# gaoxiang12/ORB-YGZ-SLAM

Hardware: AMD Instinct MI355X
Metric: frames/s ORB extract+match, 752x480 8-lvl 1000-feat; 1->8 GPU scaling (higher is better)
Workload: dtype u8

## Files before the change

### include/ygzf.h

```cpp
#ifndef YGZF_H
#define YGZF_H
#include <stddef.h>
#include <stdint.h>

#ifdef __cplusplus
extern "C" {
#endif

typedef enum ygzf_status {
    YGZF_OK = 0,
    YGZF_ERR_INVALID = -1,
    YGZF_ERR_NO_DEVICE = -2,
    YGZF_ERR_HIP = -3,
    YGZF_ERR_UNSUPPORTED = -4,
    YGZF_ERR_STATE = -5
} ygzf_status;

typedef struct ygzf_ctx ygzf_ctx;

typedef struct ygzf_extractor_cfg {
    int nfeatures;
    float scale_factor;
    int nlevels;
    int ini_th_fast;
    int min_th_fast;
    int cv_mode;
} ygzf_extractor_cfg;

typedef enum ygzf_cv_mode { YGZF_CV_LEGACY_SSE2 = 0, YGZF_CV_LEGACY_INT = 1, YGZF_CV_4 = 2 } ygzf_cv_mode;

typedef struct ygzf_kp {
    float x, y, size, angle, response;
    int32_t octave, class_id;
} ygzf_kp;

int ygzf_create(int device, const ygzf_extractor_cfg *cfg, int max_width, int max_height, int max_batch, ygzf_ctx **out);
void ygzf_destroy(ygzf_ctx *ctx);
const char *ygzf_last_error(const ygzf_ctx *ctx);

int ygzf_scale_tables_host(const ygzf_extractor_cfg *cfg, float *scale, float *inv_scale, float *sigma2, float *inv_sigma2, int *nfeat);
int ygzf_pyramid_plan_host(const ygzf_extractor_cfg *cfg, int w, int h, int *n_strips, int *lds_bytes, int *level_wh, unsigned short *rows, int rows_cap);
int ygzf_pyramid_plan_base_host(const ygzf_extractor_cfg *cfg, int w, int h);
int ygzf_octree_sort_plan_host(const ygzf_extractor_cfg *cfg, int w, int h, int *groups, int groups_cap);

int ygzf_extract_resident(ygzf_ctx *ctx, ygzf_kp *kps, uint8_t *desc, int cap, int *n_out);

int ygzf_device_mem_info(ygzf_ctx *ctx, size_t *free_bytes, size_t *total_bytes);

enum ygzf_fast_plan { YGZF_FAST_PLAN_AUTO = 0, YGZF_FAST_PLAN_ONE_PASS = 1, YGZF_FAST_PLAN_INI_FIRST = 2 };
int ygzf_set_fast_plan(ygzf_ctx *ctx, int plan);
int ygzf_get_fast_plan(const ygzf_ctx *ctx, int *plan);
enum ygzf_fast_kernel { YGZF_FAST_KERNEL_AUTO = 0, YGZF_FAST_KERNEL_REGISTER_STAGING = 1, YGZF_FAST_KERNEL_CELL_TABLE = 2 };
int ygzf_set_fast_kernel(ygzf_ctx *ctx, int kernel);
int ygzf_get_fast_stats(const ygzf_ctx *ctx, float *corner_quads_per_pass, float *passes_per_cell);
int ygzf_phase_clocks(ygzf_ctx *ctx, int kernel, unsigned long long *out16, int reset);
int ygzf_set_extract_ahead(ygzf_ctx *ctx, int on);
int ygzf_set_carry_previous(ygzf_ctx *ctx, int on);

int ygzf_get_levels(const ygzf_ctx *ctx);
int ygzf_get_scale_tables(const ygzf_ctx *ctx, float *scale, float *inv_scale, float *sigma2, float *inv_sigma2);
int ygzf_get_features_per_level(const ygzf_ctx *ctx, int *nfeat);
int ygzf_level_size(const ygzf_ctx *ctx, int w, int h, int level, int *lw, int *lh);
int ygzf_host_row_pitch(int w);
int ygzf_max_keypoints(const ygzf_ctx *ctx, int w, int h);

int ygzf_compute_pyramid(ygzf_ctx *ctx, const uint8_t *img, int w, int h, int stride, uint8_t *const *levels_out);

int ygzf_extract(ygzf_ctx *ctx, const uint8_t *img, int w, int h, int stride, ygzf_kp *kps, uint8_t *desc, int cap, int *n_out);

int ygzf_extract_batch_device(ygzf_ctx *ctx, const uint8_t *d_imgs, int n_frames, int w, int h, int row_pitch, size_t frame_stride);
int ygzf_extract_batch_host(ygzf_ctx *ctx, const uint8_t *imgs, int n_frames, int w, int h, int row_pitch, size_t frame_stride);
int ygzf_extract_batch_host_frames(ygzf_ctx *ctx, const uint8_t *const *frames, int n_frames, int w, int h, int row_pitch);
int ygzf_batch_counts(ygzf_ctx *ctx, int *n_kp );
int ygzf_batch_fetch(ygzf_ctx *ctx, int frame, ygzf_kp *kps, uint8_t *desc, int cap, int *n_out);
int ygzf_batch_fetch_all(ygzf_ctx *ctx, ygzf_kp *kps, uint8_t *desc, int *n_kp, int stride);
int ygzf_batch_fetch_packed(ygzf_ctx *ctx, void *host, size_t host_bytes, size_t *off_kps, size_t *off_desc, int *row_entries, size_t *bytes_out);
// ... 187 lines not shown
```

### orb_ygz_slam_amd/capi.py

```python
import ctypes as C
import os

import numpy as np

from . import build as _build

KP_DTYPE = np.dtype([("x", "<f4"), ("y", "<f4"), ("size", "<f4"), ("angle", "<f4"), ("response", "<f4"),
                     ("octave", "<i4"), ("class_id", "<i4")])
assert KP_DTYPE.itemsize == 28


class YgzfError(RuntimeError):
    pass


class ExtractorCfg(C.Structure):
    _fields_ = [("nfeatures", C.c_int), ("scale_factor", C.c_float), ("nlevels", C.c_int), ("ini_th_fast", C.c_int),
                ("min_th_fast", C.c_int), ("cv_mode", C.c_int)]


CV_LEGACY_SSE2, CV_LEGACY_INT, CV_4 = 0, 1, 2


class Camera(C.Structure):
# ... 193 lines not shown
def host_row_pitch(w):
    return load_library().ygzf_host_row_pitch(int(w))


def pyramid_plan_host(nfeatures, scale_factor, nlevels, w, h):
    L = load_library()
    cfg = ExtractorCfg(nfeatures, scale_factor, nlevels, 20, 7, 0)
    n, lds = C.c_int(0), C.c_int(0)
    wh = np.zeros(2 * nlevels, np.int32)
    rows = np.zeros(64 * nlevels * 4, np.uint16)
    rc = L.ygzf_pyramid_plan_host(C.byref(cfg), w, h, C.byref(n), C.byref(lds), _p(wh), _p(rows), rows.size)
    if rc != 0:
        raise YgzfError("ygzf_pyramid_plan_host failed (%d)" % rc)
    L.ygzf_pyramid_plan_base_host.argtypes = [C.c_void_p, C.c_int, C.c_int]
    base = L.ygzf_pyramid_plan_base_host(C.byref(cfg), w, h)
    if base < 0:
        raise YgzfError("ygzf_pyramid_plan_base_host failed (%d)" % base)
    return {"strips": n.value, "base": base, "lds_bytes": lds.value, "levels": [(int(wh[2 * l]), int(wh[2 * l + 1])) for l in range(nlevels)],
            "rows": rows[:n.value * nlevels * 4].astype(np.int64).reshape(n.value, nlevels, 4)}


def octree_sort_plan_host(nfeatures, scale_factor, nlevels, w, h):
    L = load_library()
    L.ygzf_octree_sort_plan_host.argtypes = [C.POINTER(ExtractorCfg), C.c_int, C.c_int, C.c_void_p, C.c_int]
    cfg = ExtractorCfg(nfeatures, scale_factor, nlevels, 20, 7, 0)
    out = np.zeros(6 * 16, np.int32)
    n = L.ygzf_octree_sort_plan_host(C.byref(cfg), w, h, _p(out), out.size)
    if n < 0:
        raise YgzfError("ygzf_octree_sort_plan_host failed (%d)" % n)
    keys = ("l0", "n", "block", "cap", "lds_cand", "lds_bytes")
    return [dict(zip(keys, (int(v) for v in out[6 * i:6 * i + 6]))) for i in range(n)]


class Extractor:

    def __init__(self, nfeatures=1000, scale_factor=1.2, nlevels=8, ini_th=20, min_th=7, max_width=752, max_height=480,
                 max_batch=1, device=0, cv_mode=CV_LEGACY_SSE2):
        self.L = load_library()
        self.nlevels = nlevels
        self.cfg = ExtractorCfg(nfeatures, scale_factor, nlevels, ini_th, min_th, cv_mode)
        self._wh = (max_width, max_height, 0)
        self.max_width, self.max_height = max_width, max_height
        self._inflight = []
        self.h = C.c_void_p()
        rc = self.L.ygzf_create(device, C.byref(self.cfg), max_width, max_height, max_batch, C.byref(self.h))
        if rc != 0:
            self.h = C.c_void_p()
            raise YgzfError("ygzf_create failed (%d): %s" % (rc, self.L.ygzf_last_error(None).decode()))

    def close(self):
        if getattr(self, "h", None) and self.h.value:
            self.L.ygzf_destroy(self.h)
            self.h = C.c_void_p()

    def __del__(self):
        try:
            self.close()
        except Exception:
            pass

    def _ck(self, rc):
        if rc < 0:
            raise YgzfError("libygzf error %d: %s" % (rc, self.L.ygzf_last_error(self.h).decode()))
        return rc

    def tables(self):
# ... 796 lines not shown
```

### orb_ygz_slam_amd/csrc/kernels.h

```cpp
#ifndef YGZF_KERNELS_H
#define YGZF_KERNELS_H
#include "ygzf_internal.h"

namespace ygzf {

hipError_t upload_constants(const int *umax16);

struct PyrTabs {
    const int *xofs;
    const short *xalpha;
    const int *yofs;
    const short *ybeta;
    const PyrColRec *cols;
    const PyrRowRec *rows;
    const PyrTileRec *tiles;
};
void launch_pyr_resize(hipStream_t st, const FrameSet &fs, const LevelGeom *dGeom, const LevelGeom &g, int level, int nFrames, const PyrTabs &T);
constexpr int kPyrFolds = 4;
__host__ __device__ constexpr int pyr_fold_chunks(int foldLog2) { return foldLog2 == 0 ? 21 : foldLog2 == 1 ? 11 : foldLog2 == 2 ? 6 : 3; }
__host__ __device__ constexpr int pyr_fold_pitch(int foldLog2) { return 16 * pyr_fold_chunks(foldLog2); }
__host__ __device__ constexpr int pyr_fold_rows(int foldLog2) { return foldLog2 == 0 ? 44 : foldLog2 == 1 ? 84 : foldLog2 == 2 ? 166 : 330; }
constexpr int kPyrTileRows = 32;
void launch_repitch_rows(hipStream_t st, const uint8_t *src, size_t srcPitch, uint8_t *dst, size_t dstPitch, int w, size_t rows);
constexpr int kHostFrameListMax = 128;
// ... 98 lines not shown
    const float *mpProjX, *mpProjY, *mpProjXR, *mpViewCos, *mpAngle;
    const int *mpLevel;
    float nnratio;
    int maxDist;
    float fx, fy, cx, cy, mb, mbf, minX, minY, maxX, maxY, gridInvW, gridInvH;
    float scaleFactors[kMaxLevels];
    float th;
    int bMono, checkLevel, checkOri;
    uint8_t *owner;
    int *match;
    int *nmatches;
    int *match12;
    int capCur, capLast, descInLds, qpInLds;
    int spill;
    int specDeep;
    void *spillScratch;
    long long spillStride;
    void *qpScratch;
    long long *dbg;
    int handoverFence;
    int fixedLanes;
    int unitWorld;
    int serialOrder;
    int split;
    int *splitCnt;
    unsigned char *splitX;
    unsigned *matchStat;
};
constexpr int kMatchStatFallbacks = 0, kMatchStatRoundCap = 1, kMatchStatExtRoom = 2, kMatchStatExtended = 3, kMatchStatRescans = 4, kMatchStatWords = 5;
constexpr int kMatchCauseRounds = 1, kMatchCauseExtRoom = 2;
constexpr int kSpillSpec = 1, kSpillMisc = 2;
constexpr int kMatchSplitRec = 56;
size_t match_lds_bytes(int capCur, int capLast, bool descInLds, int spill, size_t *spillBytes, bool specDeep);
hipError_t match_prepare(size_t ldsBytes);
void launch_backproject_unit(hipStream_t st, const ygzf_kp *keys, const int *cnt, long long kpStride, int maxKp, int nFrames, float fx,
                             float fy, float cx, float cy, float *world);
void launch_match_last(hipStream_t st, const MatchArgs &A, int nPairs, size_t ldsBytes);


void launch_bow(hipStream_t st, int nNodes, const int *kfOff, const int *kfIdx, const int *fOff, const int *fIdx, const uint8_t *kfValid,
                const ygzf_kp *kfKeys, const uint8_t *kfDesc, int nF, const ygzf_kp *fKeys, const uint8_t *fDesc, float nnratio, int checkOri, int *match,
                unsigned char *binOf, int *hist, int *nmatches);

struct TriArgs {
    int nEntries, nNodes, n1;
    const int *off1, *idx1, *off2, *idx2;
    const ygzf_kp *keys1, *keys2;
    const uint8_t *desc1, *desc2, *hasMp1, *hasMp2;
    const float *uR1, *uR2;
    const float *sf2, *sigma2;
    float F[9];
    float ex, ey;
    int onlyStereo, checkOri;
    int *match12;
    unsigned char *binOf;
    int *hist, *nmatches;
};
void launch_triangulation(hipStream_t st, const TriArgs &A);

struct FrustumArgs {
    int n;
    const uint8_t *candidate;
    const float *world, *normal, *maxDistInv, *minDistInv, *mfMaxDistance;
    float Rcw[9], tcw[3], Ow[3];
    float fx, fy, cx, cy, mbf, minX, minY, maxX, maxY;
    float viewingCosLimit;
// ... 167 lines not shown
```

### orb_ygz_slam_amd/csrc/match_kernels.hip

```cpp
#include "kernels.h"
#include "wave_ops.h"

namespace ygzf {

constexpr int GRID_COLS = 64, GRID_ROWS = 48, GRID_CELLS = GRID_COLS * GRID_ROWS;
constexpr int TH_HIGH = 100;
constexpr int HISTO_LENGTH = 30;

__device__ __forceinline__ int m_lane() { return threadIdx.x & 63; }

__device__ __forceinline__ int m_wave_incl_scan(int v) { return wave_incl_scan(v); }

__global__ void k_backproject_unit(const ygzf_kp *__restrict__ keys, const int *__restrict__ cnt, long long kpStride, float fx,
                                   float fy, float cx, float cy, float *__restrict__ world) {
    const int f = blockIdx.y;
    const int i = blockIdx.x * blockDim.x + threadIdx.x;
    if (i >= cnt[f]) return;
    const ygzf_kp k = keys[(long long) f * kpStride + i];
    float *w = world + ((long long) f * kpStride + i) * 3;
    w[0] = (k.x - cx) / fx;
    w[1] = (k.y - cy) / fy;
    w[2] = 1.f;
}

struct QueryParam {
    float u, v, radius, ur, angle;
    unsigned char minCx, maxCx, minCy, maxCy;
    signed char minLevel, maxLevel;
    unsigned char valid, hasObs;
    unsigned pad;
};

constexpr int kMatchBlock = 1024;
constexpr unsigned kNoKey = (256u << 16);
constexpr int kExtSlots = 64;

typedef unsigned v4u_t __attribute__((ext_vector_type(4)));
typedef __attribute__((address_space(3))) const v4u_t lds_uint4_t;
__device__ __forceinline__ void lds_desc(const unsigned long long *base, int i2, unsigned long long &d0, unsigned long long &d1, unsigned long long &d2,
                                         unsigned long long &d3) {
    lds_uint4_t *p = (lds_uint4_t *) (base + 4 * (size_t) i2);
    const v4u_t a = p[0], b = p[1];
    d0 = ((unsigned long long) a.y << 32) | a.x; d1 = ((unsigned long long) a.w << 32) | a.z;
    d2 = ((unsigned long long) b.y << 32) | b.x; d3 = ((unsigned long long) b.w << 32) | b.z;
}

struct MatchLds {
    int *cellStart, *cellFill, *list, *events;
    QueryParam *qp;
    unsigned long long *desc;
    float *cx, *cy, *cang;
    uint4 *specKey;
    ushort4 *specI2;
    uint4 *specKeyB;
    ushort4 *specI2B;
    float *qang;
    unsigned char *qobs;
    unsigned char *owner, *octave;
    int *match;
    int *claim;
    unsigned char *extOf;
    unsigned *extKey;
    unsigned short *extI2;
    int *extWork;
};

__device__ __forceinline__ unsigned wave_min_dpp(unsigned v) {
    unsigned t;
    t = (unsigned) __builtin_amdgcn_update_dpp((int) v, (int) v, 0xb1, 0xf, 0xf, false); v = t < v ? t : v;
    t = (unsigned) __builtin_amdgcn_update_dpp((int) v, (int) v, 0x4e, 0xf, 0xf, false); v = t < v ? t : v;
    t = (unsigned) __builtin_amdgcn_update_dpp((int) v, (int) v, 0x124, 0xf, 0xf, false); v = t < v ? t : v;
    t = (unsigned) __builtin_amdgcn_update_dpp((int) v, (int) v, 0x128, 0xf, 0xf, false); v = t < v ? t : v;
    const unsigned a = (unsigned) __builtin_amdgcn_readlane((int) v, 0), b = (unsigned) __builtin_amdgcn_readlane((int) v, 16);
    const unsigned c = (unsigned) __builtin_amdgcn_readlane((int) v, 32), d = (unsigned) __builtin_amdgcn_readlane((int) v, 48);
    const unsigned ab = a < b ? a : b, cd = c < d ? c : d;
    return ab < cd ? ab : cd;
}

#if (defined(__gfx950__) || defined(__gfx942__)) && !defined(YGZF_FORCE_HANDOVER_FENCE)
constexpr bool kHandoverScopedAccess = true;
#else
// ... 162 lines not shown
    for (int st = 4; st >= 1; st >>= 1)
#pragma unroll
        for (int e = 0; e < 8; e++)
            if ((e & st) == 0 && K[e + st] < K[e]) {
                const unsigned tk = K[e], tj = J[e];
                K[e] = K[e + st]; J[e] = J[e + st];
                K[e + st] = tk; J[e + st] = tj;
            }
}

template <int kXor>
__device__ __forceinline__ void spec_merge8_xor(unsigned (&K)[8], unsigned (&J)[8], int lane) {
    const int addr = (lane ^ kXor) << 2;
    unsigned pk[8], pj[8];
#pragma unroll
    for (int e = 0; e < 8; e++) {
        pk[e] = (unsigned) __builtin_amdgcn_ds_bpermute(addr, (int) K[7 - e]);
        pj[e] = (unsigned) __builtin_amdgcn_ds_bpermute(addr, (int) J[7 - e]);
    }
#pragma unroll
    for (int e = 0; e < 8; e++)
        if (pk[e] < K[e]) { K[e] = pk[e]; J[e] = pj[e]; }
#pragma unroll
    for (int st = 4; st >= 1; st >>= 1)
#pragma unroll
        for (int e = 0; e < 8; e++)
            if ((e & st) == 0 && K[e + st] < K[e]) {
                const unsigned tk = K[e], tj = J[e];
                K[e] = K[e + st]; J[e] = J[e + st];
                K[e + st] = tk; J[e + st] = tj;
            }
}

__global__ __launch_bounds__(kMatchBlock) void k_match_last(MatchArgs A) {
    extern __shared__ __attribute__((aligned(16))) unsigned char dyn[];
    __shared__ int s_tmp[20];
    __shared__ int s_hist[HISTO_LENGTH];
    const int tid = threadIdx.x, lane = m_lane(), wave = tid >> 6;
    const int S = A.split > 1 ? A.split : 1;
    const int pair = S > 1 ? (int) blockIdx.x / S : (int) blockIdx.x, part = (int) blockIdx.x - pair * S;
    const int nt = A.curCnt[(long long) pair * A.cntStrideCur + A.cntOffCur];
    const int nq = A.lastCnt[(long long) pair * A.cntStrideLast + A.cntOffLast];
    const ygzf_kp *curKeys = A.curKeys + (long long) pair * A.kpStrideCur;
    const uint8_t *curDesc = A.curDesc + (long long) pair * A.kpStrideCur * 32;
    const float *uRight = A.curURight ? A.curURight + (long long) pair * A.kpStrideCur : nullptr;
    const ygzf_kp *lastKeys = A.lastKeys + (long long) pair * A.kpStrideLast;
    const uint8_t *mpDesc = A.mpDesc + (long long) pair * A.kpStrideLast * 32;
    const float *world = A.world + (long long) pair * A.kpStrideLast * 3;
    const uint8_t *mpValid = A.mpValid ? A.mpValid + (long long) pair * A.kpStrideLast : nullptr;
    const uint8_t *outlier = A.outlier ? A.outlier + (long long) pair * A.kpStrideLast : nullptr;
    const uint8_t *hasObs = A.hasObs ? A.hasObs + (long long) pair * A.kpStrideLast : nullptr;
    uint8_t *ownerOut = A.owner + (long long) pair * A.kpStrideCur;
    int *matchOut = A.match + (long long) pair * A.kpStrideCur;
    const float *pose = A.poses + (long long) pair * 24;

    long long *dbg = A.dbg ? A.dbg + (long long) pair * 8 : nullptr;
#define STAMP(k) do { if (dbg && tid == 0) dbg[k] = wall_clock64(); } while (0)
    const long long tStart = dbg ? wall_clock64() : 0;
    MatchLds L;
    unsigned char *p = dyn;
    unsigned char *gp = (unsigned char *) A.spillScratch + (long long) pair * A.spillStride;
#define CARVE(ptr, type, count, bit)                                                        \
    do {                                                                                    \
        if (A.spill & (bit)) { ptr = (type *) gp; gp += (((size_t) sizeof(type) * (count)) + 15) & ~(size_t) 15; } \
        else { ptr = (type *) p; p += (((size_t) sizeof(type) * (count)) + 15) & ~(size_t) 15; }                   \
    } while (0)
    CARVE(L.cellStart, int, GRID_CELLS + 1, 0);
    CARVE(L.cellFill, int, GRID_CELLS, 0);
    CARVE(L.list, int, A.capCur, 0);
    CARVE(L.cx, float, A.capCur, 0);
    CARVE(L.cy, float, A.capCur, 0);
    CARVE(L.owner, unsigned char, A.capCur, 0);
    CARVE(L.octave, unsigned char, A.capCur, 0);
    CARVE(L.qobs, unsigned char, A.capLast, 0);
    CARVE(L.specKey, uint4, A.capLast, kSpillSpec);
    CARVE(L.specI2, ushort4, A.capLast, kSpillSpec);
    L.specKeyB = nullptr;
    L.specI2B = nullptr;
    if (A.specDeep) {
        CARVE(L.specKeyB, uint4, A.capLast, kSpillSpec);
        CARVE(L.specI2B, ushort4, A.capLast, kSpillSpec);
    }
    CARVE(L.events, int, A.capLast, kSpillMisc);
    CARVE(L.qang, float, A.capLast, kSpillMisc);
    CARVE(L.cang, float, A.capCur, kSpillMisc);
    CARVE(L.match, int, A.capCur, kSpillMisc);
    CARVE(L.claim, int, A.capCur, kSpillMisc);
    CARVE(L.extOf, unsigned char, 2 * (size_t) A.capLast, kSpillMisc);
    CARVE(L.extKey, unsigned, 8 * kExtSlots, kSpillMisc);
    CARVE(L.extI2, unsigned short, 8 * kExtSlots, kSpillMisc);
    CARVE(L.extWork, int, kExtSlots, kSpillMisc);
    L.desc = nullptr;
    if (A.descInLds) CARVE(L.desc, unsigned long long, 4 * (size_t) A.capCur, 0);
#undef CARVE
    L.qp = (QueryParam *) A.qpScratch + (long long) pair * A.capLast;

    for (int i = tid; i < GRID_CELLS; i += kMatchBlock) L.cellFill[i] = 0;
    if (tid < HISTO_LENGTH) s_hist[tid] = 0;
    __syncthreads();
    for (int i = tid; i < nt; i += kMatchBlock) {
        const ygzf_kp k = curKeys[i];
        const int px = (int) roundf((k.x - A.minX) * A.gridInvW);
        const int py = (int) roundf((k.y - A.minY) * A.gridInvH);
        if (!(px < 0 || px >= GRID_COLS || py < 0 || py >= GRID_ROWS)) atomicAdd(&L.cellFill[px * GRID_ROWS + py], 1);
        L.owner[i] = A.ownerIn ? A.ownerIn[(long long) pair * A.kpStrideCur + i] : 0;
        L.octave[i] = (unsigned char) k.octave;
        L.cx[i] = k.x; L.cy[i] = k.y; L.cang[i] = k.angle;
        L.match[i] = -1;
        L.claim[i] = 64;
        if (A.descInLds) {
            const unsigned long long *d = (const unsigned long long *) (curDesc + (size_t) i * 32);
            L.desc[4 * i] = d[0]; L.desc[4 * i + 1] = d[1]; L.desc[4 * i + 2] = d[2]; L.desc[4 * i + 3] = d[3];
        }
    }
    __syncthreads();
    {
        const int per = GRID_CELLS / kMatchBlock;
        int s = 0;
        for (int k = 0; k < per; k++) s += L.cellFill[tid * per + k];
        int incl = m_wave_incl_scan(s);
        if (lane == 63) s_tmp[wave] = incl;
        __syncthreads();
        int woff = 0;
        for (int w2 = 0; w2 < wave; w2++) woff += s_tmp[w2];
        int off = woff + incl - s;
        for (int k = 0; k < per; k++) {
            const int c = L.cellFill[tid * per + k];
            L.cellStart[tid * per + k] = off;
            off += c;
        }
        if (tid == kMatchBlock - 1) L.cellStart[GRID_CELLS] = off;
    }
    __syncthreads();
    for (int i = tid; i < GRID_CELLS; i += kMatchBlock) L.cellFill[i] = L.cellStart[i];
    __syncthreads();
    for (int i = tid; i < nt; i += kMatchBlock) {
        const int px = (int) roundf((L.cx[i] - A.minX) * A.gridInvW);
        const int py = (int) roundf((L.cy[i] - A.minY) * A.gridInvH);
        if (!(px < 0 || px >= GRID_COLS || py < 0 || py >= GRID_ROWS)) L.list[atomicAdd(&L.cellFill[px * GRID_ROWS + py], 1)] = i;
    }
    __syncthreads();
    for (int c = tid; c < GRID_CELLS; c += kMatchBlock) {
        const int s = L.cellStart[c], e = L.cellStart[c + 1];
        for (int a = s + 1; a < e; a++) {
            const int v = L.list[a];
            int b = a - 1;
            while (b >= s && L.list[b] > v) { L.list[b + 1] = L.list[b]; b--; }
            L.list[b + 1] = v;
        }
    }
    __syncthreads();
    const long long tGrid = dbg ? wall_clock64() : 0;
    const float *Rcw = pose, *tcw = pose + 9, *Rlw = pose + 12, *tlw = pose + 21;
    float twc[3], tlc2;
    for (int i = 0; i < 3; i++) twc[i] = -1 * (Rcw[i] * tcw[0] + Rcw[3 + i] * tcw[1] + Rcw[6 + i] * tcw[2]);
    tlc2 = (Rlw[6] * twc[0] + Rlw[7] * twc[1] + Rlw[8] * twc[2]) + tlw[2];
    const bool bForward = tlc2 > A.mb && !A.bMono;
    const bool bBackward = -tlc2 > A.mb && !A.bMono;
    const int nLocal = (nq - part + S - 1) / S;
    int LPQ = S > 1 ? 8 : 1, qr = S > 1 ? (tid & 7) : 0;
    int jFirst = S > 1 ? (tid >> 3) : tid, jStep = S > 1 ? (kMatchBlock >> 3) : kMatchBlock, jEnd = nLocal;
    if (nLocal <= kMatchBlock && !A.fixedLanes) {
        const int nUse = min(kMatchBlock / 64, max(4, (nLocal * 8 + 63) / 64));
        int jb, je;
        if (nLocal <= 32) {
            jb = nLocal * min(wave, nUse) / nUse;
            je = nLocal * min(wave + 1, nUse) / nUse;
        } else {
        int *wsum = L.events;
        int wgt = 0;
        if (tid < nLocal) {
            const int i = tid * S + part;
            int lvl = (A.mode == 0 || A.mode == 3) ? lastKeys[i].octave : A.mpLevel[(long long) pair * A.kpStrideLast + i];
            lvl = min(max(lvl, 0), (int) kMaxLevels - 1);
// ... 1391 lines not shown
    for (int i = p0 + wave; i < p1; i += kMatchBlock / 64) {
        const size_t o = ((size_t) R.out + (size_t) i) * (size_t) nBest;
        if (skip && skip[i]) {
            if (lane == 0)
                for (int k = 0; k < nBest; k++) { A.bestIdx[o + k] = -1; A.bestDist[o + k] = 256; }
            continue;
        }
        proj_search_point<MODE>(K, R.R2, R.t2, keys, kdesc, uRight, keyMatched, cellStart, list, world + 3 * (size_t) i,
                                normal ? normal + 3 * (size_t) i : nullptr, minInv[i], maxInv[i], mfMax[i],
                                (const uint64_t *) (mpDesc + 32 * (size_t) i), A.th, nBest, A.maxHamming, lane, A.bestIdx + o, A.bestDist + o);
    }
}

template <int MODE>
static hipError_t launch_proj_mode(hipStream_t st, const ProjArgs &A, int maxKeys) {
    hipError_t e = hipFuncSetAttribute((const void *) k_proj_search<MODE>, hipFuncAttributeMaxDynamicSharedMemorySize, kMaxDynLds);
    if (e != hipSuccess) return e;
    hipLaunchKernelGGL(k_proj_search<MODE>, dim3((A.maxPoints + A.slice - 1) / A.slice, A.nRows), dim3(kMatchBlock), fuse_lds_bytes(maxKeys), st, A);
    return hipSuccess;
}

hipError_t launch_proj_search(hipStream_t st, const ProjArgs &A, int maxKeys) {
    if (A.nRows <= 0 || A.maxPoints <= 0) return hipSuccess;
    switch (A.mode) {
    case PM_FUSE: return launch_proj_mode<PM_FUSE>(st, A, maxKeys);
    case PM_FUSE_SCW: return launch_proj_mode<PM_FUSE_SCW>(st, A, maxKeys);
    case PM_PROJ_SCW: return launch_proj_mode<PM_PROJ_SCW>(st, A, maxKeys);
    case PM_SIM3: return launch_proj_mode<PM_SIM3>(st, A, maxKeys);
    }
    return hipErrorInvalidValue;
}

size_t match_lds_bytes(int capCur, int capLast, bool descInLds, int spill, size_t *spillBytes, bool specDeep) {
    size_t lds = al16(sizeof(int) * (GRID_CELLS + 1)) + al16(sizeof(int) * GRID_CELLS) + al16(sizeof(int) * (size_t) capCur) +
                 2 * al16(sizeof(float) * (size_t) capCur) + 2 * al16((size_t) capCur) + al16((size_t) capLast);
    size_t gl = 0;
    const size_t spec = (specDeep ? 2 : 1) * (al16(sizeof(uint4) * (size_t) capLast) + al16(sizeof(ushort4) * (size_t) capLast));
    const size_t misc = al16(sizeof(int) * (size_t) capLast) + al16(sizeof(float) * (size_t) capLast) + al16(sizeof(float) * (size_t) capCur) +
                        2 * al16(sizeof(int) * (size_t) capCur) + al16(2 * (size_t) capLast) + al16(sizeof(unsigned) * 8 * kExtSlots) +
                        al16(sizeof(unsigned short) * 8 * kExtSlots) + al16(sizeof(int) * kExtSlots);
    if (spill & kSpillSpec) gl += spec; else lds += spec;
    if (spill & kSpillMisc) gl += misc; else lds += misc;
    if (descInLds) lds += al16((size_t) 32 * capCur);
    if (spillBytes) *spillBytes = gl;
    return lds + 64;
}

hipError_t match_prepare(size_t ldsBytes) {
    return hipFuncSetAttribute((const void *) k_match_last, hipFuncAttributeMaxDynamicSharedMemorySize, kMaxDynLds);
}

void launch_backproject_unit(hipStream_t st, const ygzf_kp *keys, const int *cnt, long long kpStride, int maxKp, int nFrames, float fx,
                             float fy, float cx, float cy, float *world) {
    if (maxKp <= 0) return;
    hipLaunchKernelGGL(k_backproject_unit, dim3((maxKp + 255) / 256, nFrames), dim3(256), 0, st, keys, cnt, kpStride, fx, fy, cx, cy, world);
}

void launch_match_last(hipStream_t st, const MatchArgs &A, int nPairs, size_t ldsBytes) {
    hipLaunchKernelGGL(k_match_last, dim3(nPairs * (A.split > 1 ? A.split : 1)), dim3(kMatchBlock), ldsBytes, st, A);
}

}
```

### orb_ygz_slam_amd/csrc/ygzf_api_match.hip

```cpp
#include "ygzf_ctx.h"

extern "C" {

static void grid_inverses(const ygzf_camera &cam, float &invW, float &invH) {
    invW = (float) 64 / (cam.max_x - cam.min_x);
    invH = (float) 48 / (cam.max_y - cam.min_y);
}

static void fill_camera(MatchArgs &A, const ygzf_camera *cam, const ygzf_ctx *c) {
    A.fx = cam->fx; A.fy = cam->fy; A.cx = cam->cx; A.cy = cam->cy; A.mb = cam->mb; A.mbf = cam->mbf;
    A.minX = cam->min_x; A.minY = cam->min_y; A.maxX = cam->max_x; A.maxY = cam->max_y;
    grid_inverses(*cam, A.gridInvW, A.gridInvH);
    for (int l = 0; l < kMaxLevels; l++) A.scaleFactors[l] = l < c->tab.cfg.nlevels ? c->tab.scale[l] : 1.f;
}
static void fill_view_scales(MatchArgs &A, const ygzf_frame_view *F) {
    if (F->scale_factors) for (int l = 0; l < kMaxLevels && l < F->nlevels; l++) A.scaleFactors[l] = F->scale_factors[l];
}

static int plan_match_lds(ygzf_ctx *c, MatchArgs &A, int nPairs, size_t *ldsBytes) {
    const size_t budget = 156 * 1024;
    if (A.capCur > 65535) return fail(c, YGZF_ERR_UNSUPPORTED, "matcher supports at most 65535 keypoints per frame");
    A.qpInLds = 0;
    const struct { int desc, spill; } plans[] = {{1, 0}, {0, 0}, {0, kSpillSpec}, {0, kSpillSpec | kSpillMisc}};
    size_t b = 0, sp = 0;
    bool ok = false;
    for (const auto &pl : plans) {
        b = match_lds_bytes(A.capCur, A.capLast, pl.desc != 0, pl.spill, &sp, A.specDeep != 0);
        if (b <= budget) { A.descInLds = pl.desc; A.spill = pl.spill; ok = true; break; }
    }
    if (!ok) return fail(c, YGZF_ERR_UNSUPPORTED, "matcher needs %zu bytes of LDS for %d/%d keypoints", b, A.capCur, A.capLast);
    int rc = ensure(c, c->dQp, (size_t) nPairs * A.capLast * 32);
    if (rc) return rc;
    A.qpScratch = c->dQp.p;
    A.spillStride = (long long) sp;
    A.spillScratch = nullptr;
    if (sp) {
        if ((rc = ensure(c, c->dSpill, (size_t) nPairs * sp))) return rc;
        A.spillScratch = c->dSpill.p;
    }
    if (!c->dMatchStat.p) {
        if ((rc = ensure(c, c->dMatchStat, 64))) return rc;
        HIPCHECK(c, hipMemsetAsync(c->dMatchStat.p, 0, 64, c->stream));
    }
    A.matchStat = (unsigned *) c->dMatchStat.p;
    A.serialOrder = c->matchSerial;
    A.handoverFence = c->matchFence;
    A.fixedLanes = c->matchFixedLanes;
    A.split = 1;
    A.splitCnt = nullptr;
    A.splitX = nullptr;
    if (!A.spill && A.capLast >= 128 && c->matchSplit != 1) {
        int sp2 = c->matchSplit > 1 ? c->matchSplit : 256 / (nPairs > 0 ? nPairs : 1);
        sp2 = std::min(sp2, c->matchSplit > 1 ? 128 : 64);
        if (sp2 > 1) {
            const size_t cntBytes = (size_t) nPairs * sizeof(int);
            if (c->dSplitCnt.bytes < cntBytes) {
                if ((rc = ensure(c, c->dSplitCnt, cntBytes > 4096 ? cntBytes : 4096))) return rc;
                HIPCHECK(c, hipMemsetAsync(c->dSplitCnt.p, 0, c->dSplitCnt.bytes, c->stream));
            }
            if ((rc = ensure(c, c->dSplitX, (size_t) nPairs * A.capLast * kMatchSplitRec))) return rc;
            A.split = sp2;
            A.splitCnt = (int *) c->dSplitCnt.p;
            A.splitX = (unsigned char *) c->dSplitX.p;
// ... 104 lines not shown
    A.world = (const float *) c->dWorld.p;
    A.lastCnt = cnt;
    A.kpStrideLast = G.kpStride;
    A.cntStrideLast = 1;
    A.cntOffLast = 0;
    A.poses = (const float *) c->dPoses.p;
    fill_camera(A, cam, c);
    A.th = th;
    A.bMono = b_mono != 0;
    A.checkLevel = check_level != 0;
    A.checkOri = check_orientation != 0;
    A.owner = (uint8_t *) c->dOwner.p;
    A.match = (int *) c->dMatch.p;
    A.nmatches = (int *) c->dNMatch.p;
    A.capCur = G.kpStride;
    A.capLast = G.kpStride;
    if ((rc = run_match(c, A, B, B > 1 ? 1 : 0, B > 1 ? "pair 1" : "pair 0"))) return rc;
    set_match_pairs(c, B);
    return YGZF_OK;
}

static int read_match_stats(ygzf_ctx *c, unsigned *dst, int words) {
    if (!c || !dst) return fail(c, YGZF_ERR_INVALID, "null argument");
    for (int i = 0; i < words; i++) dst[i] = 0;
    if (!c->dMatchStat.p) return YGZF_OK;
    HIPCHECK(c, hipSetDevice(c->device));
    HIPCHECK(c, hipMemcpyAsync(dst, c->dMatchStat.p, words * sizeof(unsigned), hipMemcpyDeviceToHost, c->stream));
    HIPCHECK(c, hipStreamSynchronize(c->stream));
    return YGZF_OK;
}
int ygzf_match_fallbacks(ygzf_ctx *c, unsigned *pairs) { return read_match_stats(c, pairs, 1); }
int ygzf_match_path_stats(ygzf_ctx *c, unsigned stats[5]) { return read_match_stats(c, stats, kMatchStatWords); }

int ygzf_match_counts(ygzf_ctx *c, int *nmatches) {
    if (!c || !nmatches) return fail(c, YGZF_ERR_INVALID, "null argument");
    if (c->held.matchPairs < 1) return fail(c, YGZF_ERR_STATE, "no matched batch");
    HIPCHECK(c, hipMemcpyAsync(nmatches, c->dNMatch.p, sizeof(int) * c->held.matchPairs, hipMemcpyDeviceToHost, c->stream));
    HIPCHECK(c, hipStreamSynchronize(c->stream));
    return YGZF_OK;
}

int ygzf_match_fetch(ygzf_ctx *c, int frame, int *cur_match, uint8_t *cur_owner, int cap) {
    if (!c) return fail(c, YGZF_ERR_INVALID, "null argument");
    if (c->held.matchPairs < 1) return fail(c, YGZF_ERR_STATE, "no matched batch");
    if (frame < 0 || frame >= c->held.matchPairs) return fail(c, YGZF_ERR_INVALID, "frame %d out of range", frame);
    int n = 0;
    HIPCHECK(c, hipMemcpyAsync(&n, (int *) c->dOutCnt.p + frame + 1, sizeof(int), hipMemcpyDeviceToHost, c->stream));
    HIPCHECK(c, hipStreamSynchronize(c->stream));
    if (n > cap) return fail(c, YGZF_ERR_INVALID, "capacity %d < %d keypoints", cap, n);
    const size_t base = (size_t) frame * c->geo.kpStride;
    if (cur_match && n) HIPCHECK(c, hipMemcpyAsync(cur_match, (int *) c->dMatch.p + base, sizeof(int) * n, hipMemcpyDeviceToHost, c->stream));
    if (cur_owner && n) HIPCHECK(c, hipMemcpyAsync(cur_owner, (uint8_t *) c->dOwner.p + base, n, hipMemcpyDeviceToHost, c->stream));
    HIPCHECK(c, hipStreamSynchronize(c->stream));
    return YGZF_OK;
}

int ygzf_match_fetch_all(ygzf_ctx *c, int *match, int stride) {
    if (!c || !match) return fail(c, YGZF_ERR_INVALID, "null argument");
    if (c->held.matchPairs < 1) return fail(c, YGZF_ERR_STATE, "no matched batch");
    const int B = c->held.matchPairs, ks = c->geo.kpStride;
    if (stride < ks) return fail(c, YGZF_ERR_INVALID, "stride %d < %d (ygzf_max_keypoints)", stride, ks);
    HIPCHECK(c, hipMemcpy2DAsync(match, sizeof(int) * (size_t) stride, c->dMatch.p, sizeof(int) * (size_t) ks, sizeof(int) * (size_t) ks, B,
                                 hipMemcpyDeviceToHost, c->stream));
    HIPCHECK(c, hipStreamSynchronize(c->stream));
    return YGZF_OK;
}
// ... 802 lines not shown
```

### orb_ygz_slam_amd/csrc/ygzf_ctx.h

```cpp
#ifndef YGZF_CTX_H
#define YGZF_CTX_H
#include <cmath>
#include <cstdarg>
#include <cstdio>
#include <cstdlib>
#include <cstring>
#include <limits>
#include <mutex>

#include "kernels.h"

#define YGZF_HIDDEN __attribute__((visibility("hidden")))

namespace ygzf {
YGZF_HIDDEN int cv_round_host(double v);
enum KernelKind { KK_PYR = 0, KK_FAST, KK_OCTREE, KK_DESCRIBE, KK_HAMMING, KK_BACKPROJ, KK_MATCH, KK_SIA, KK_FAST10, KK_DSO, KK_STEREO, KK_DIRECT, KK_BOW, KK_FRUSTUM, KK_DISTINCTIVE, KK_BOWNODES, KK_GRID, KK_FASTQ, KK_TRI, KK_FASTP, KK_FUSE, KK_PROJ, KK_COUNT };
static const char *kKernelNames[KK_COUNT] = {"k_pyr_resize", "k_fast_tab", "k_octree", "k_describe", "k_hamming_pairs",
                                             "k_backproject_unit", "k_match_last", "k_sia_run", "k_f10_*", "k_dso_cells", "k_stereo_*", "k_direct_projection", "k_bow_descend", "k_frustum", "k_distinctive", "k_bow_nodes", "k_features_in_area", "k_fast_quads", "k_tri_nodes", "k_fast_tab_persist", "k_fuse", "k_proj_search"};

struct Geometry {
    int w = 0, h = 0;
    std::vector<LevelGeom> lv;
    std::vector<int> xofs, yofs;
    std::vector<short> xalpha, ybeta;
// ... 84 lines not shown
    unsigned *hFastStats = nullptr;
    Buf dFastCtr;
    int cuCount = 256;
    Buf dResPack;
    Buf dUpStage;
    hipEvent_t evShare = nullptr;
    hipEvent_t evPyrDone = nullptr;
    uint8_t *hIn = nullptr;
    void *hInDev = nullptr;
    size_t hInBytes = 0;
    hipEvent_t evIn = nullptr;
    bool evInPending = false;
    uint8_t *hStage = nullptr;
    size_t hStageBytes = 0;
    void *hStageDev = nullptr;
    Held held;
    int img0Pitch = 0;
    hipEvent_t tStart = nullptr, tStop = nullptr;
    bool useGraphs = !debug_flag("nograph");
    int pyrStripFrames = (int) forced("pyr_strip_frames", 16);
    PyrChainGraph pyrGraph = {};
    const void *pyrGraphKey[6] = {nullptr};
    bool extractAhead = false;
    hipStream_t streamCopy = nullptr;
    hipEvent_t evPyramid = nullptr;
    bool profile = false;
    bool debugSync = debug_flag("sync");
    bool linkKernels = forced("fetch_kernel", 1) != 0, pyrLink = forced("pyr_link", 1) != 0;
    int uploadKernelFrames = (int) forced("upload_kernel_frames", 2);
    size_t uploadKernelBytes = (size_t) forced("upload_kernel_bytes", 16l << 20);
    int octHelpersForced = (int) forced("oct_helpers", -1), octHelperSpin = (int) forced("oct_helper_spin", 1 << 16);
    int fastPersistMode = (int) forced("fast_persist", -1), fastPersistWgs = (int) forced("fast_persist_wgs", 8);
    int matchSplit = (int) forced("match_split", 0);
    int matchFixedLanes = forced_is("match_lanes", "fixed");
    int matchFence = (int) forced("match_fence", 0);
    int matchSerial = (int) forced("match_serial", 0);
    bool siaPerLevel = forced("sia_precompute", 1) != 0;
    bool octDebug = debug_flag("oct"), matchDebug = debug_flag("match"), siaDebug = debug_flag("sia");
    struct Rec { int kind; hipEvent_t a, b; };
    std::vector<Rec> recs;
    std::vector<hipEvent_t> pool;
    float profMs[KK_COUNT] = {0};
    int profN[KK_COUNT] = {0};
};

extern YGZF_HIDDEN thread_local std::string g_create_err;

static int fail(ygzf_ctx *c, int code, const char *fmt, ...) {
    char buf[512];
    va_list ap;
    va_start(ap, fmt);
    vsnprintf(buf, sizeof buf, fmt, ap);
    va_end(ap);
    if (c) {
        if (c->stream) (void) hipStreamSynchronize(c->stream);
        c->err = buf;
    } else {
        g_create_err = buf;
    }
    return code;
}

#define HIPCHECK(c, expr)                                                                                         \
    do {                                                                                                          \
        hipError_t _e = (expr);                                                                                   \
        if (_e != hipSuccess) return fail(c, YGZF_ERR_HIP, "%s failed: %s (%s:%d)", #expr, hipGetErrorString(_e), \
// ... 208 lines not shown
```

Before: 259,200.

## Shrink matcher LDS footprint by aliasing cellFill and narrowing cellStart

```diff
diff --git a/include/ygzf.h b/include/ygzf.h
--- a/include/ygzf.h
+++ b/include/ygzf.h
@@ -42,6 +42,8 @@
 int ygzf_pyramid_plan_host(const ygzf_extractor_cfg *cfg, int w, int h, int *n_strips, int *lds_bytes, int *level_wh, unsigned short *rows, int rows_cap);
 int ygzf_pyramid_plan_base_host(const ygzf_extractor_cfg *cfg, int w, int h);
 int ygzf_octree_sort_plan_host(const ygzf_extractor_cfg *cfg, int w, int h, int *groups, int groups_cap);
+int ygzf_match_lds_plan_host(const ygzf_extractor_cfg *cfg, int w, int h, int cap_cur, int cap_last, int n_pairs, int spec_deep, int forced_plan,
+                             int batched_budget, long long *out, int out_cap);
 
 int ygzf_extract_resident(ygzf_ctx *ctx, ygzf_kp *kps, uint8_t *desc, int cap, int *n_out);
 
diff --git a/orb_ygz_slam_amd/capi.py b/orb_ygz_slam_amd/capi.py
--- a/orb_ygz_slam_amd/capi.py
+++ b/orb_ygz_slam_amd/capi.py
@@ -249,6 +249,25 @@
     return [dict(zip(keys, (int(v) for v in out[6 * i:6 * i + 6]))) for i in range(n)]
 
 
+MATCH_LDS_ARRAYS = ("cellStart", "cellFill", "list", "cx", "cy", "owner", "octave", "qobs", "specKey", "specI2", "specKeyB", "specI2B", "events", "qang",
+                    "cang", "match", "claim", "extOf", "extKey", "extI2", "extWork", "desc")
+
+
+def match_lds_plan_host(nfeatures, scale_factor, nlevels, w, h, cap_cur, cap_last, n_pairs, spec_deep=False, forced_plan=-1, batched_budget=False):
+    L = load_library()
+    L.ygzf_match_lds_plan_host.argtypes = [C.POINTER(ExtractorCfg)] + [C.c_int] * 8 + [C.c_void_p, C.c_int]
+    cfg = ExtractorCfg(nfeatures, scale_factor, nlevels, 20, 7, 0)
+    out = np.zeros(10 + 32, np.int64)
+    rc = L.ygzf_match_lds_plan_host(C.byref(cfg), w, h, cap_cur, cap_last, n_pairs, int(spec_deep), forced_plan, int(batched_budget), _p(out), out.size)
+    if rc not in (0, -4):
+        raise YgzfError("ygzf_match_lds_plan_host failed (%d)" % rc)
+    v = [int(x) for x in out]
+    n = v[9]
+    assert n <= len(MATCH_LDS_ARRAYS)
+    return {"plan": v[0] if rc == 0 else None, "desc": v[1], "spill": v[2], "lds_bytes": v[3], "spill_bytes": v[4], "budget": v[5], "kind_budget": v[6],
+            "fast_lds_bytes": v[7], "fill_host": v[8], "arrays": dict(zip(MATCH_LDS_ARRAYS[:n], v[10:10 + n]))}
+
+
 class Extractor:
 
     def __init__(self, nfeatures=1000, scale_factor=1.2, nlevels=8, ini_th=20, min_th=7, max_width=752, max_height=480,
diff --git a/orb_ygz_slam_amd/csrc/kernels.h b/orb_ygz_slam_amd/csrc/kernels.h
--- a/orb_ygz_slam_amd/csrc/kernels.h
+++ b/orb_ygz_slam_amd/csrc/kernels.h
@@ -154,6 +154,7 @@
 constexpr int kSpillSpec = 1, kSpillMisc = 2;
 constexpr int kMatchSplitRec = 56;
 size_t match_lds_bytes(int capCur, int capLast, bool descInLds, int spill, size_t *spillBytes, bool specDeep);
+int match_lds_carve(int capCur, int capLast, bool descInLds, int spill, bool specDeep, long long *bytes, int cap, int *fillHost);
 hipError_t match_prepare(size_t ldsBytes);
 void launch_backproject_unit(hipStream_t st, const ygzf_kp *keys, const int *cnt, long long kpStride, int maxKp, int nFrames, float fx,
                              float fy, float cx, float cy, float *world);
diff --git a/orb_ygz_slam_amd/csrc/match_kernels.hip b/orb_ygz_slam_amd/csrc/match_kernels.hip
--- a/orb_ygz_slam_amd/csrc/match_kernels.hip
+++ b/orb_ygz_slam_amd/csrc/match_kernels.hip
@@ -46,7 +46,8 @@
 }
 
 struct MatchLds {
-    int *cellStart, *cellFill, *list, *events;
+    unsigned short *cellStart;
+    int *cellFill, *list, *events;
     QueryParam *qp;
     unsigned long long *desc;
     float *cx, *cy, *cang;
@@ -275,6 +276,37 @@
             }
 }
 
+constexpr int kFillOwn = 0, kFillSpec = 1, kFillDesc = 2;
+__host__ __device__ constexpr size_t m_al16(size_t b) { return (b + 15) & ~(size_t) 15; }
+__host__ __device__ inline int match_fill_host(int capCur, int capLast, bool descInLds, int spill) {
+    const size_t need = m_al16(sizeof(int) * GRID_CELLS);
+    if (!(spill & kSpillSpec)) return m_al16(sizeof(uint4) * (size_t) capLast) + m_al16(sizeof(ushort4) * (size_t) capLast) >= need ? kFillSpec : kFillOwn;
+    return descInLds && m_al16((size_t) 32 * capCur) >= need ? kFillDesc : kFillOwn;
+}
+#define YGZF_MATCH_ARRAYS(X, capCur, capLast, fillHost, specDeep, descInLds)                          \
+    X(cellStart, unsigned short, GRID_CELLS + 1, 0, 0)                                                \
+    X(cellFill, int, (fillHost) == kFillOwn ? GRID_CELLS : 0, 0, 0)                                   \
+    X(list, int, capCur, 0, 0)                                                                        \
+    X(cx, float, capCur, 0, 0)                                                                        \
+    X(cy, float, capCur, 0, 0)                                                                        \
+    X(owner, unsigned char, capCur, 0, 0)                                                             \
+    X(octave, unsigned char, capCur, 0, 0)                                                            \
+    X(qobs, unsigned char, capLast, 0, 0)                                                             \
+    X(specKey, uint4, capLast, kSpillSpec, kFillSpec)    \
+    X(specI2, ushort4, capLast, kSpillSpec, 0)                                                        \
+    X(specKeyB, uint4, (specDeep) ? (capLast) : 0, kSpillSpec, 0)                                     \
+    X(specI2B, ushort4, (specDeep) ? (capLast) : 0, kSpillSpec, 0)                                    \
+    X(events, int, capLast, kSpillMisc, 0)                                                            \
+    X(qang, float, capLast, kSpillMisc, 0)                                                            \
+    X(cang, float, capCur, kSpillMisc, 0)                                                             \
+    X(match, int, capCur, kSpillMisc, 0)                                                              \
+    X(claim, int, capCur, kSpillMisc, 0)    \
+    X(extOf, unsigned char, 2 * (size_t) (capLast), kSpillMisc, 0)                                    \
+    X(extKey, unsigned, 8 * kExtSlots, kSpillMisc, 0)                                                 \
+    X(extI2, unsigned short, 8 * kExtSlots, kSpillMisc, 0)                                            \
+    X(extWork, int, kExtSlots, kSpillMisc, 0)                                                         \
+    X(desc, unsigned long long, (descInLds) ? 4 * (size_t) (capCur) : 0, 0, kFillDesc)
+
 __global__ __launch_bounds__(kMatchBlock) void k_match_last(MatchArgs A) {
     extern __shared__ __attribute__((aligned(16))) unsigned char dyn[];
     __shared__ int s_tmp[20];
@@ -303,39 +335,23 @@
     MatchLds L;
     unsigned char *p = dyn;
     unsigned char *gp = (unsigned char *) A.spillScratch + (long long) pair * A.spillStride;
-#define CARVE(ptr, type, count, bit)                                                        \
+    const int fillHost = match_fill_host(A.capCur, A.capLast, A.descInLds != 0, A.spill);
+    int *fillOver = nullptr;
+#define CARVE(name, type, count, bit, hostId)                                               \
     do {                                                                                    \
-        if (A.spill & (bit)) { ptr = (type *) gp; gp += (((size_t) sizeof(type) * (count)) + 15) & ~(size_t) 15; } \
-        else { ptr = (type *) p; p += (((size_t) sizeof(type) * (count)) + 15) & ~(size_t) 15; }                   \
-    } while (0)
-    CARVE(L.cellStart, int, GRID_CELLS + 1, 0);
-    CARVE(L.cellFill, int, GRID_CELLS, 0);
-    CARVE(L.list, int, A.capCur, 0);
-    CARVE(L.cx, float, A.capCur, 0);
-    CARVE(L.cy, float, A.capCur, 0);
-    CARVE(L.owner, unsigned char, A.capCur, 0);
-    CARVE(L.octave, unsigned char, A.capCur, 0);
-    CARVE(L.qobs, unsigned char, A.capLast, 0);
-    CARVE(L.specKey, uint4, A.capLast, kSpillSpec);
-    CARVE(L.specI2, ushort4, A.capLast, kSpillSpec);
-    L.specKeyB = nullptr;
-    L.specI2B = nullptr;
-    if (A.specDeep) {
-        CARVE(L.specKeyB, uint4, A.capLast, kSpillSpec);
-        CARVE(L.specI2B, ushort4, A.capLast, kSpillSpec);
-    }
-    CARVE(L.events, int, A.capLast, kSpillMisc);
-    CARVE(L.qang, float, A.capLast, kSpillMisc);
-    CARVE(L.cang, float, A.capCur, kSpillMisc);
-    CARVE(L.match, int, A.capCur, kSpillMisc);
-    CARVE(L.claim, int, A.capCur, kSpillMisc);
-    CARVE(L.extOf, unsigned char, 2 * (size_t) A.capLast, kSpillMisc);
-    CARVE(L.extKey, unsigned, 8 * kExtSlots, kSpillMisc);
-    CARVE(L.extI2, unsigned short, 8 * kExtSlots, kSpillMisc);
-    CARVE(L.extWork, int, kExtSlots, kSpillMisc);
-    L.desc = nullptr;
-    if (A.descInLds) CARVE(L.desc, unsigned long long, 4 * (size_t) A.capCur, 0);
+        const size_t nb = m_al16((size_t) sizeof(type) * (count));                          \
+        if (A.spill & (bit)) { L.name = (type *) gp; gp += nb; }                            \
+        else {                                                                              \
+            if ((hostId) != 0 && fillHost == (hostId)) fillOver = (int *) p;                \
+            L.name = (type *) p; p += nb;                                                   \
+        }                                                                                   \
+    } while (0);
+    YGZF_MATCH_ARRAYS(CARVE, A.capCur, A.capLast, fillHost, A.specDeep, A.descInLds)
 #undef CARVE
+    if (fillHost != kFillOwn) L.cellFill = fillOver;
+    if (!A.specDeep) { L.specKeyB = nullptr; L.specI2B = nullptr; }
+    if (!A.descInLds) L.desc = nullptr;
+    const bool descAfterGrid = fillHost == kFillDesc;
     L.qp = (QueryParam *) A.qpScratch + (long long) pair * A.capLast;
 
     for (int i = tid; i < GRID_CELLS; i += kMatchBlock) L.cellFill[i] = 0;
@@ -351,7 +367,7 @@
         L.cx[i] = k.x; L.cy[i] = k.y; L.cang[i] = k.angle;
         L.match[i] = -1;
         L.claim[i] = 64;
-        if (A.descInLds) {
+        if (A.descInLds && !descAfterGrid) {
             const unsigned long long *d = (const unsigned long long *) (curDesc + (size_t) i * 32);
             L.desc[4 * i] = d[0]; L.desc[4 * i + 1] = d[1]; L.desc[4 * i + 2] = d[2]; L.desc[4 * i + 3] = d[3];
         }
@@ -369,10 +385,10 @@
         int off = woff + incl - s;
         for (int k = 0; k < per; k++) {
             const int c = L.cellFill[tid * per + k];
-            L.cellStart[tid * per + k] = off;
+            L.cellStart[tid * per + k] = (unsigned short) off;
             off += c;
         }
-        if (tid == kMatchBlock - 1) L.cellStart[GRID_CELLS] = off;
+        if (tid == kMatchBlock - 1) L.cellStart[GRID_CELLS] = (unsigned short) off;
     }
     __syncthreads();
     for (int i = tid; i < GRID_CELLS; i += kMatchBlock) L.cellFill[i] = L.cellStart[i];
@@ -383,6 +399,11 @@
         if (!(px < 0 || px >= GRID_COLS || py < 0 || py >= GRID_ROWS)) L.list[atomicAdd(&L.cellFill[px * GRID_ROWS + py], 1)] = i;
     }
     __syncthreads();
+    if (descAfterGrid)
+        for (int i = tid; i < nt; i += kMatchBlock) {
+            const unsigned long long *d = (const unsigned long long *) (curDesc + (size_t) i * 32);
+            L.desc[4 * i] = d[0]; L.desc[4 * i + 1] = d[1]; L.desc[4 * i + 2] = d[2]; L.desc[4 * i + 3] = d[3];
+        }
     for (int c = tid; c < GRID_CELLS; c += kMatchBlock) {
         const int s = L.cellStart[c], e = L.cellStart[c + 1];
         for (int a = s + 1; a < e; a++) {
@@ -1840,18 +1861,23 @@
 }
 
 size_t match_lds_bytes(int capCur, int capLast, bool descInLds, int spill, size_t *spillBytes, bool specDeep) {
-    size_t lds = al16(sizeof(int) * (GRID_CELLS + 1)) + al16(sizeof(int) * GRID_CELLS) + al16(sizeof(int) * (size_t) capCur) +
-                 2 * al16(sizeof(float) * (size_t) capCur) + 2 * al16((size_t) capCur) + al16((size_t) capLast);
-    size_t gl = 0;
-    const size_t spec = (specDeep ? 2 : 1) * (al16(sizeof(uint4) * (size_t) capLast) + al16(sizeof(ushort4) * (size_t) capLast));
-    const size_t misc = al16(sizeof(int) * (size_t) capLast) + al16(sizeof(float) * (size_t) capLast) + al16(sizeof(float) * (size_t) capCur) +
-                        2 * al16(sizeof(int) * (size_t) capCur) + al16(2 * (size_t) capLast) + al16(sizeof(unsigned) * 8 * kExtSlots) +
-                        al16(sizeof(unsigned short) * 8 * kExtSlots) + al16(sizeof(int) * kExtSlots);
-    if (spill & kSpillSpec) gl += spec; else lds += spec;
-    if (spill & kSpillMisc) gl += misc; else lds += misc;
-    if (descInLds) lds += al16((size_t) 32 * capCur);
+    const int fillHost = match_fill_host(capCur, capLast, descInLds, spill);
+    size_t lds = 0, gl = 0;
+#define SIZE(name, type, count, bit, hostId) { const size_t nb = m_al16((size_t) sizeof(type) * (count)); if (spill & (bit)) gl += nb; else lds += nb; }
+    YGZF_MATCH_ARRAYS(SIZE, capCur, capLast, fillHost, specDeep, descInLds)
+#undef SIZE
     if (spillBytes) *spillBytes = gl;
     return lds + 64;
+}
+
+int match_lds_carve(int capCur, int capLast, bool descInLds, int spill, bool specDeep, long long *bytes, int cap, int *fillHostOut) {
+    const int fillHost = match_fill_host(capCur, capLast, descInLds, spill);
+    int n = 0;
+#define SIZE(name, type, count, bit, hostId) { const long long nb = (long long) m_al16((size_t) sizeof(type) * (count)); if (n < cap) bytes[n] = (spill & (bit)) ? -nb : nb; n++; }
+    YGZF_MATCH_ARRAYS(SIZE, capCur, capLast, fillHost, specDeep, descInLds)
+#undef SIZE
+    if (fillHostOut) *fillHostOut = fillHost;
+    return n;
 }
 
 hipError_t match_prepare(size_t ldsBytes) {
diff --git a/orb_ygz_slam_amd/csrc/ygzf_api_match.hip b/orb_ygz_slam_amd/csrc/ygzf_api_match.hip
--- a/orb_ygz_slam_amd/csrc/ygzf_api_match.hip
+++ b/orb_ygz_slam_amd/csrc/ygzf_api_match.hip
@@ -17,18 +17,40 @@
     if (F->scale_factors) for (int l = 0; l < kMaxLevels && l < F->nlevels; l++) A.scaleFactors[l] = F->scale_factors[l];
 }
 
+static const struct { int desc, spill; } kMatchPlans[] = {{1, 0}, {0, 0}, {1, kSpillSpec}, {0, kSpillSpec}, {0, kSpillSpec | kSpillMisc}};
+constexpr int kMatchPlanCount = (int) (sizeof kMatchPlans / sizeof kMatchPlans[0]);
+constexpr size_t kMatchLdsWide = 156 * 1024;
+constexpr int kMatchBatchedPairs = 128;
+
+static size_t match_lds_budget(const Geometry &G, int nPairs, int matchSplit, bool batchedBudget) {
+    if (!batchedBudget || nPairs <= kMatchBatchedPairs || matchSplit > 1) return kMatchLdsWide;
+    const size_t fast = 4 * fast_tab_lds_bytes(G.fastWinRows, G.fastSmapRows, G.fastQuadCap);
+    return fast < (size_t) 160 * 1024 ? std::min((size_t) 160 * 1024 - fast, kMatchLdsWide) : 0;
+}
+
+struct MatchLdsPlan { int index; size_t bytes, spillBytes, budget; };
+static bool choose_match_plan(int capCur, int capLast, bool specDeep, size_t budget, int forcedPlan, MatchLdsPlan &P) {
+    P.index = -1; P.bytes = P.spillBytes = 0;
+    if (forcedPlan >= kMatchPlanCount) return false;
+    for (const size_t bud : {budget, kMatchLdsWide}) {
+        P.budget = forcedPlan >= 0 ? kMatchLdsWide : bud;
+        for (int k = forcedPlan >= 0 ? forcedPlan : 0; k < (forcedPlan >= 0 ? forcedPlan + 1 : kMatchPlanCount); k++) {
+            P.bytes = match_lds_bytes(capCur, capLast, kMatchPlans[k].desc != 0, kMatchPlans[k].spill, &P.spillBytes, specDeep);
+            if (P.bytes <= P.budget) { P.index = k; return true; }
+        }
+    }
+    return false;
+}
+
 static int plan_match_lds(ygzf_ctx *c, MatchArgs &A, int nPairs, size_t *ldsBytes) {
-    const size_t budget = 156 * 1024;
     if (A.capCur > 65535) return fail(c, YGZF_ERR_UNSUPPORTED, "matcher supports at most 65535 keypoints per frame");
     A.qpInLds = 0;
-    const struct { int desc, spill; } plans[] = {{1, 0}, {0, 0}, {0, kSpillSpec}, {0, kSpillSpec | kSpillMisc}};
-    size_t b = 0, sp = 0;
-    bool ok = false;
-    for (const auto &pl : plans) {
-        b = match_lds_bytes(A.capCur, A.capLast, pl.desc != 0, pl.spill, &sp, A.specDeep != 0);
-        if (b <= budget) { A.descInLds = pl.desc; A.spill = pl.spill; ok = true; break; }
-    }
-    if (!ok) return fail(c, YGZF_ERR_UNSUPPORTED, "matcher needs %zu bytes of LDS for %d/%d keypoints", b, A.capCur, A.capLast);
+    MatchLdsPlan P;
+    if (!choose_match_plan(A.capCur, A.capLast, A.specDeep != 0, match_lds_budget(c->geo, nPairs, c->matchSplit, c->matchBatchedBudget), c->matchLdsPlan, P))
+        return fail(c, YGZF_ERR_UNSUPPORTED, "matcher needs %zu bytes of LDS for %d/%d keypoints", P.bytes, A.capCur, A.capLast);
+    A.descInLds = kMatchPlans[P.index].desc;
+    A.spill = kMatchPlans[P.index].spill;
+    const size_t b = P.bytes, sp = P.spillBytes;
     int rc = ensure(c, c->dQp, (size_t) nPairs * A.capLast * 32);
     if (rc) return rc;
     A.qpScratch = c->dQp.p;
@@ -199,6 +221,30 @@
 int ygzf_match_fallbacks(ygzf_ctx *c, unsigned *pairs) { return read_match_stats(c, pairs, 1); }
 int ygzf_match_path_stats(ygzf_ctx *c, unsigned stats[5]) { return read_match_stats(c, stats, kMatchStatWords); }
 
+int ygzf_match_lds_plan_host(const ygzf_extractor_cfg *cfg, int w, int h, int cap_cur, int cap_last, int n_pairs, int spec_deep, int forced_plan,
+                             int batched_budget, long long *out, int out_cap) {
+    if (!cfg || cfg->nlevels < 1 || cfg->nlevels > kMaxLevels || cfg->nfeatures < 0 || !(cfg->scale_factor > 1.0f) || w < 1 || h < 1 || cap_cur < 0 ||
+        cap_cur > 65535 || cap_last < 0 || n_pairs < 1 || !out || out_cap < 10)
+        return YGZF_ERR_INVALID;
+    ygzf_ctx tmp;
+    tmp.tab.init(*cfg);
+    Geometry G;
+    const int rc = build_geometry(&tmp, w, h, G);
+    if (rc) return rc;
+    MatchLdsPlan P;
+    const size_t kind = match_lds_budget(G, n_pairs, 0, batched_budget != 0);
+    const bool ok = choose_match_plan(cap_cur, cap_last, spec_deep != 0, kind, forced_plan, P);
+    for (int i = 0; i < out_cap; i++) out[i] = 0;
+    out[0] = P.index; out[3] = (long long) P.bytes; out[4] = (long long) P.spillBytes; out[5] = (long long) P.budget; out[6] = (long long) kind;
+    out[7] = (long long) fast_tab_lds_bytes(G.fastWinRows, G.fastSmapRows, G.fastQuadCap);
+    if (!ok) return YGZF_ERR_UNSUPPORTED;
+    out[1] = kMatchPlans[P.index].desc; out[2] = kMatchPlans[P.index].spill;
+    int fillHost = 0;
+    out[9] = match_lds_carve(cap_cur, cap_last, out[1] != 0, (int) out[2], spec_deep != 0, out + 10, out_cap - 10, &fillHost);
+    out[8] = fillHost;
+    return YGZF_OK;
+}
+
 int ygzf_match_counts(ygzf_ctx *c, int *nmatches) {
     if (!c || !nmatches) return fail(c, YGZF_ERR_INVALID, "null argument");
     if (c->held.matchPairs < 1) return fail(c, YGZF_ERR_STATE, "no matched batch");
diff --git a/orb_ygz_slam_amd/csrc/ygzf_ctx.h b/orb_ygz_slam_amd/csrc/ygzf_ctx.h
--- a/orb_ygz_slam_amd/csrc/ygzf_ctx.h
+++ b/orb_ygz_slam_amd/csrc/ygzf_ctx.h
@@ -140,6 +140,8 @@
     int octHelpersForced = (int) forced("oct_helpers", -1), octHelperSpin = (int) forced("oct_helper_spin", 1 << 16);
     int fastPersistMode = (int) forced("fast_persist", -1), fastPersistWgs = (int) forced("fast_persist_wgs", 8);
     int matchSplit = (int) forced("match_split", 0);
+    int matchLdsPlan = (int) forced("match_lds", -1);
+    bool matchBatchedBudget = forced("match_batched_budget", 0) != 0;
     int matchFixedLanes = forced_is("match_lanes", "fixed");
     int matchFence = (int) forced("match_fence", 0);
     int matchSerial = (int) forced("match_serial", 0);
```

Measured after the change: 260,000, median of 6. No clear change (+0.3%).
